# apple/ml-neuman

Hardware: AMD Instinct MI355X
Metric: rays_per_sec (800x800 frame, 128 samples/ray coarse + 128 importance, NeuMan background NeRF) (higher is better)
Workload: dtype coarse (sampling) pass: split-fp16 hi+lo MFMA x3, f32 accumulate; fine (shading) pass: per-row-scaled int16 as two int8 limbs on the i8 MFMA x3, exact int32 accumulate, encodings on split bf16

## Files before the change

ml-neuman_amd/csrc/mlp_device.h:

```cpp
#pragma once
#include "common.h"
#include "mlp_layout.h"
#include "mlp_launch.h"

namespace {

using nm::kTileM;

typedef __attribute__((ext_vector_type(8))) __bf16 bf16x8;
typedef __attribute__((ext_vector_type(2))) __bf16 bf16x2;
typedef __attribute__((ext_vector_type(8))) _Float16 f16x8;
typedef __attribute__((ext_vector_type(2))) _Float16 f16x2;

constexpr bool is_split(int prec) { return prec == NM_PREC_BF16X3 || prec == NM_PREC_FP16X3; }
constexpr float kF16ActScale = 32.f;
typedef __attribute__((ext_vector_type(2))) float f32x2;
typedef __attribute__((ext_vector_type(16))) float f32x16;

constexpr int kThreads = 512;
constexpr int kChunkU4 = 2 * kTileM;
constexpr int kLoU4 = kTileM;
constexpr int H_BASE = 0;
constexpr int P_BASE = nm::kHChunks * kChunkU4;
constexpr int LDS_U4 = P_BASE + nm::kPeChunks * kChunkU4;
// ... 17 lines not shown
    float* out;
    float* dbg;
    unsigned long long* prof;
    int64_t n;
    int S;
    int in_mode;
    const int* ray_idx;
    const int* n_rays_dev;
    int s0, S_total;
    int stop_stage;
    float sigma_scale;
    int sigma_only;
    PeSpec pos, dir;
    float* save_h;
    float* save_hv;
    unsigned* save_bits;
    uint4* save_h16;
    uint4* save_feat16;
    unsigned* save_hvbits;
    uint4* save_x0h;
    uint4* save_d0h;
};

__device__ __forceinline__ float pe_feature(int p, float x0, float x1, float x2, PeSpec spec, const float* __restrict__ tab) {
    const int m = p - 3;
    float a = 0.f;
    bool is_cos = false;
    if (p >= 3 && m < 6 * spec.nfreq) {
        if (spec.kind == NM_PE_POSENC) {
            const int b = m / 6, r = m - 6 * b;
            const int dim = r >= 3 ? r - 3 : r;
            const float xv = dim == 0 ? x0 : (dim == 1 ? x1 : x2);
            a = xv * tab[b];
            is_cos = r >= 3;
        } else {
            const int n3 = 3 * spec.nfreq;
            is_cos = m >= n3;
            const float* b = tab + 3 * (is_cos ? m - n3 : m);
            a = fmaf(x2, b[2], fmaf(x1, b[1], x0 * b[0]));
        }
    }
    float sv, cv;
    sincosf(a, &sv, &cv);
    if (p < 3) return p == 0 ? x0 : (p == 1 ? x1 : x2);
    if (m >= 6 * spec.nfreq) return 0.f;
    return is_cos ? cv : sv;
}

__device__ __forceinline__ int64_t sample_record(const MlpArgs& a, int64_t i) {
    if (a.in_mode >= 3) return a.ray_idx[i];
    if (a.in_mode != 2) return i;
    const int64_t j = i / a.S;
    return (int64_t)a.ray_idx[j] * a.S_total + a.s0 + (i - j * a.S);
}
__device__ __forceinline__ void sample_input(const MlpArgs& a, int64_t i, bool is_dir, float& x0, float& x1, float& x2) {
    if (a.in_mode == 0 || a.in_mode == 4) {
        if (a.in_mode == 4) i = a.ray_idx[i];
        const float* src = (is_dir ? a.dirs : a.pts) + i * 3;
        x0 = src[0]; x1 = src[1]; x2 = src[2];
        return;
    }
    int64_t r, zi;
    if (a.in_mode == 3) i = a.ray_idx[i];
    if (a.in_mode != 2) {
        r = i / a.S;
        zi = i;
    } else {
        const int64_t j = i / a.S;
        r = a.ray_idx[j];
        zi = r * a.S_total + a.s0 + (i - j * a.S);
    }
    const float* d = a.direction + r * 3;
    if (is_dir) {
        x0 = d[0]; x1 = d[1]; x2 = d[2];
    } else {
        const float zz = a.z[zi];
        const float* o = a.origin + r * 3;
        x0 = o[0] + d[0] * zz;
        x1 = o[1] + d[1] * zz;
        x2 = o[2] + d[2] * zz;
    }
}

template <bool RELU, bool F16 = false>
__device__ __forceinline__ void split8(const float* v, uint4& hi, uint4& lo, float scale = 1.f) {
    unsigned h[4], l[4];
#pragma unroll
    for (int p = 0; p < 4; ++p) {
        f32x2 a = {v[2 * p], v[2 * p + 1]};
        if (F16) {
            a.x = __builtin_amdgcn_fmed3f(a.x * scale, RELU ? 0.f : -65504.f, 65504.f);
            a.y = __builtin_amdgcn_fmed3f(a.y * scale, RELU ? 0.f : -65504.f, 65504.f);
            const f16x2 hb = __builtin_convertvector(a, f16x2);
            const f32x2 hf = __builtin_convertvector(hb, f32x2);
            const f32x2 r = {a.x - hf.x, a.y - hf.y};
            const f16x2 lb = __builtin_convertvector(r, f16x2);
            h[p] = __builtin_bit_cast(unsigned, hb);
            l[p] = __builtin_bit_cast(unsigned, lb);
            continue;
        }
        if (RELU) {
            a.x = fmaxf(a.x, 0.f);
            a.y = fmaxf(a.y, 0.f);
        }
        const bf16x2 hb = __builtin_convertvector(a, bf16x2);
        const f32x2 hf = __builtin_convertvector(hb, f32x2);
        const f32x2 r = {a.x - hf.x, a.y - hf.y};
        const bf16x2 lb = __builtin_convertvector(r, bf16x2);
        h[p] = __builtin_bit_cast(unsigned, hb);
        l[p] = __builtin_bit_cast(unsigned, lb);
    }
    hi = make_uint4(h[0], h[1], h[2], h[3]);
    lo = make_uint4(l[0], l[1], l[2], l[3]);
}

__device__ __forceinline__ bf16x8 as_bf16x8(uint4 v) { return __builtin_bit_cast(bf16x8, v); }

typedef __attribute__((vector_size(16))) unsigned int v4u;
__device__ __forceinline__ bf16x8 ld_w(__amdgpu_buffer_rsrc_t wsrc, int voff, int soff) {
    return __builtin_bit_cast(bf16x8, __builtin_amdgcn_raw_buffer_load_b128(wsrc, voff, soff, 0));
}

struct WPre {
    bf16x8 h[2], l[2];
};
template <int PREC>
__device__ __forceinline__ void w_prefetch(WPre& W, __amdgpu_buffer_rsrc_t wsrc, int voff, int soff) {
#pragma unroll
    for (int u = 0; u < 2; ++u) {
        W.h[u] = ld_w(wsrc, voff, soff + u * nm::kStepBytes);
        if (is_split(PREC)) W.l[u] = ld_w(wsrc, voff, soff + u * nm::kStepBytes + 1024);
    }
}

template <int MB, int PREC>
__device__ __forceinline__ void x_load(uint4 (&h)[MB], uint4 (&l)[MB], const uint4* ph) {
#pragma unroll
    for (int mb = 0; mb < MB; ++mb) {
        h[mb] = ph[mb * 32];
        if (is_split(PREC)) l[mb] = ph[kLoU4 + mb * 32];
    }
}
__device__ __forceinline__ f16x8 as_f16x8(uint4 v) { return __builtin_bit_cast(f16x8, v); }
template <int MB, int PREC>
__device__ __forceinline__ void mfma_step(f32x16 (&acc)[MB], bf16x8 wh, bf16x8 wl, const uint4 (&xh)[MB], const uint4 (&xl)[MB]) {
    if (PREC == NM_PREC_FP16X3) {
        const f16x8 fh = __builtin_bit_cast(f16x8, wh), fl = __builtin_bit_cast(f16x8, wl);
#pragma unroll
        for (int mb = 0; mb < MB; ++mb) acc[mb] = __builtin_amdgcn_mfma_f32_32x32x16_f16(fh, as_f16x8(xl[mb]), acc[mb], 0, 0, 0);
#pragma unroll
        for (int mb = 0; mb < MB; ++mb) acc[mb] = __builtin_amdgcn_mfma_f32_32x32x16_f16(fl, as_f16x8(xh[mb]), acc[mb], 0, 0, 0);
#pragma unroll
        for (int mb = 0; mb < MB; ++mb) acc[mb] = __builtin_amdgcn_mfma_f32_32x32x16_f16(fh, as_f16x8(xh[mb]), acc[mb], 0, 0, 0);
        return;
    }
    if (PREC == NM_PREC_BF16X3) {
#pragma unroll
        for (int mb = 0; mb < MB; ++mb) acc[mb] = __builtin_amdgcn_mfma_f32_32x32x16_bf16(wh, as_bf16x8(xl[mb]), acc[mb], 0, 0, 0);
#pragma unroll
        for (int mb = 0; mb < MB; ++mb) acc[mb] = __builtin_amdgcn_mfma_f32_32x32x16_bf16(wl, as_bf16x8(xh[mb]), acc[mb], 0, 0, 0);
    }
#pragma unroll
    for (int mb = 0; mb < MB; ++mb) acc[mb] = __builtin_amdgcn_mfma_f32_32x32x16_bf16(wh, as_bf16x8(xh[mb]), acc[mb], 0, 0, 0);
}
template <int MB, int PREC>
__device__ __forceinline__ void k_run(f32x16 (&acc)[MB], WPre& W, __amdgpu_buffer_rsrc_t wsrc, int voff, int soff, int next_soff,
// ... 211 lines not shown
```

ml-neuman_amd/csrc/mlp_f16t.hip:

```cpp
#include "mlp_i8as.h"
#include <stdio.h>
#include <stdlib.h>

namespace {

constexpr int kWavesF = 4;
constexpr int kTileF = kWavesF * kRows;
constexpr int kPosU4F = nm::kPeChunks * 2 * kRows;
constexpr int kPeF = kWavesF * kPosU4F;
constexpr int kStepU4F = nm::kStepBytes / 16;
constexpr int kSlotU4F = 16 * kStepU4F;
constexpr int kSlotsF = 3;
constexpr int kF16TabF = 2 * nm::kStages + 2;
constexpr int kTabU4F = (nm::kBiasFloats + kF16TabF + 3) / 4;
constexpr int kSigmaStepsF = 8 * 4 + 6 * 8 * 16 + 8 * 20 + 16;
static_assert((kPeF + kSlotsF * kSlotU4F + kTabU4F) * 16 <= 160 * 1024, "LDS plan exceeds the CU");

struct RingF {
    const char* src;
    const uint4* rd;
    unsigned lds0;
    int off;
    int slot;
};
__device__ __forceinline__ void ring_piece_f(const RingF& R, int off, int slot, int j) {
    glds16(R.src + off + j * (kWavesF * 1024), __builtin_amdgcn_readfirstlane(R.lds0 + slot * (kSlotU4F * 16) + j * (kWavesF * 1024)));
}

struct ArgsF {
    MlpArgs a;
    const uint4* stream;
    const float* bias16;
    unsigned* dbg;
    int dbg_stage;
    int64_t dbg_tile;
};

#ifdef NM_F16T_BODY
#include NM_F16T_BODY
#else
#include "mlp_f16t_body.h"
#endif

__global__ __launch_bounds__(kWavesF * 64) __attribute__((amdgpu_waves_per_eu(1, 1))) void nerf_sigma_f16t_kernel(const ArgsF A) {
    __shared__ uint4 lds[kPeF + kSlotsF * kSlotU4F + kTabU4F];
    const MlpArgs a = resolve_args(A.a);
    const int tid = threadIdx.x, lane = tid & 63;
    const int w = __builtin_amdgcn_readfirstlane(tid >> 6);
    const int g = lane >> 5, s = lane & 31;
    uint4* pw = lds + w * kPosU4F;
    RingF R;
    R.src = reinterpret_cast<const char*>(A.stream) + lane * 16 + w * 1024;
    R.rd = lds + kPeF + lane;
    R.lds0 = (unsigned)(uintptr_t)(lds + kPeF) + w * 1024;
    {
        float* lb = reinterpret_cast<float*>(lds + kPeF + kSlotsF * kSlotU4F);
        for (int i = tid; i < nm::kBiasFloats + kF16TabF; i += kWavesF * 64) lb[i] = A.bias16[i];
    }
    for (int i = lane; i < kPosU4F; i += 64) pw[i] = make_uint4(0, 0, 0, 0);
    __syncthreads();
    for (int j = 0; j < kF16tUnit0Pieces; ++j) ring_piece_f(R, 0, 0, j);
    for (int j = 0; j < kF16tUnit0Pieces; ++j) ring_piece_f(R, kF16tUnit0Pieces * 4096, 1, j);
    R.off = 2 * kF16tUnit0Pieces * 4096;
    if (kF16tUnit0Pieces == 4) asm volatile("s_waitcnt vmcnt(4)" ::: "memory");
    else if (kF16tUnit0Pieces == 3) asm volatile("s_waitcnt vmcnt(3)" ::: "memory");
    else asm volatile("s_waitcnt vmcnt(2)" ::: "memory");
    __syncthreads();
    R.slot = 1;
    const float os = A.bias16[nm::kBiasFloats + nm::kStages + 8];
    unsigned bias_lds = (unsigned)(uintptr_t)(lds + kPeF + kSlotsF * kSlotU4F) + 16 * g;
    asm volatile("" : "+v"(bias_lds));
    const unsigned tab_lds = (unsigned)(uintptr_t)(lds + kPeF + kSlotsF * kSlotU4F) + nm::kBiasFloats * 4;
    const int64_t ntiles = (a.n + kTileF - 1) / kTileF;
#pragma unroll 1
    for (int64_t tile = blockIdx.x; tile < ntiles; tile += gridDim.x) {
        const int64_t row0 = tile * kTileF + w * kRows;
        fill_pe_wave<true>(pw, false, a, row0, lane);
        sigma_stages_asm(A, a, R, pw, bias_lds, tab_lds, g, s, tid, tile, row0, os);
    }
    asm volatile("s_waitcnt vmcnt(0)" ::: "memory");
}

}

namespace nm {

int sigma_f16t_ndir() { return kF16tNdir; }

int launch_sigma_f16t(const MlpLaunch& L, const void* stream16t, int stream_ndir, const float* pts, const float* dirs, const float* origin, const float* direction,
                      const float* z, int64_t n, int S, int in_mode, float sigma_scale, float* out, hipStream_t stream, const MlpChunk* chunk,
                      float* dbg, int dbg_stage) {
    static_assert(kSigmaStepsF * kStepBytes == 976 * 2048, "stream length");
    NM_REQUIRE(stream_ndir == kF16tNdir, "nerf_sigma_f16t_kernel: the stream was cut for %d direct parts per k-step, the kernel is generated for %d", stream_ndir, kF16tNdir);
    ArgsF A;
    MlpArgs& a = A.a;
    a.ray_idx = chunk ? chunk->ray_idx : nullptr;
    a.n_rays_dev = chunk ? chunk->n_rays_dev : nullptr;
    a.s0 = chunk ? chunk->s0 : 0;
    a.S_total = chunk ? chunk->S_total : S;
    a.wpack = nullptr; a.bias = nullptr;
    a.petab = L.petab;
    a.pts = pts; a.dirs = dirs; a.origin = origin; a.direction = direction; a.z = z;
    a.out = out; a.dbg = nullptr; a.prof = nullptr; a.n = n; a.S = S; a.in_mode = in_mode; a.stop_stage = -2; a.sigma_scale = sigma_scale;
    a.sigma_only = 1;
    a.save_h = nullptr; a.save_hv = nullptr; a.save_bits = nullptr; a.save_h16 = nullptr; a.save_feat16 = nullptr; a.save_hvbits = nullptr; a.save_x0h = nullptr; a.save_d0h = nullptr;
    a.pos = PeSpec{L.pe_kind, L.pos_nfreq, L.pos_octaves};
    a.dir = PeSpec{L.pe_kind, L.dir_nfreq, L.dir_octaves};
    A.stream = reinterpret_cast<const uint4*>(stream16t);
    A.bias16 = L.bias16;
    A.dbg = reinterpret_cast<unsigned*>(dbg);
    A.dbg_stage = dbg ? dbg_stage % 100 : -1;
    A.dbg_tile = dbg ? (int64_t)(dbg_stage / 100) * 256 : -1;
    const int64_t ntiles = (n + kTileF - 1) / kTileF;
    int dev = 0, cus = 256;
    if (hipGetDevice(&dev) == hipSuccess) {
        int v = 0;
        if (hipDeviceGetAttribute(&v, hipDeviceAttributeMultiprocessorCount, dev) == hipSuccess && v > 0) cus = v;
    }
    const int grid = (int)(ntiles < cus ? ntiles : cus);
    hipLaunchKernelGGL(nerf_sigma_f16t_kernel, dim3(grid), dim3(kWavesF * 64), 0, stream, A);
    return check_launch("nerf_sigma_f16t_kernel");
}

}
```

ml-neuman_amd/csrc/mlp_i8as.h:

```cpp
#pragma once
#include "mlp_device.h"

namespace {

typedef __attribute__((ext_vector_type(4))) int i32x4;
typedef __attribute__((ext_vector_type(16))) int i32x16;
typedef __attribute__((ext_vector_type(2))) short i16x2;
typedef __attribute__((address_space(3))) const float lds_cfloat;
typedef __attribute__((ext_vector_type(4))) float vf4;
typedef __attribute__((address_space(3))) const vf4 lds_cvf4;

constexpr int kRows = 32;
struct Args8s {
    MlpArgs a;
    const float* consts8;
    const uint4* image8;
    nm::LiveList live;
};

__device__ __forceinline__ i32x4 as_i32x4(uint4 v) { return __builtin_bit_cast(i32x4, v); }

template <bool F16 = false>
__device__ __forceinline__ void fill_pe_wave(uint4* pw, bool is_dir, const MlpArgs& a, int64_t base_row, int lane) {
    const PeSpec spec = is_dir ? a.dir : a.pos;
    const float* tab = a.petab + (is_dir ? 96 : 0);
    unsigned short* hi = reinterpret_cast<unsigned short*>(pw);
    auto put = [&](int row, int p, float v, bool clamp = false) {
        const int off = ((p >> 3) * (2 * kRows) + row) * 8 + (p & 7);
        if (F16) {
            float sv = v * kF16ActScale;
            if (clamp) sv = __builtin_amdgcn_fmed3f(sv, -65504.f, 65504.f);
            const _Float16 hb = (_Float16)sv;
            const _Float16 lb = (_Float16)(sv - (float)hb);
            hi[off] = __builtin_bit_cast(unsigned short, hb);
            hi[off + kRows * 8] = __builtin_bit_cast(unsigned short, lb);
            return;
        }
        const bf16x2 hb = __builtin_convertvector((f32x2){v, 0.f}, bf16x2);
        const f32x2 hf = __builtin_convertvector(hb, f32x2);
        const bf16x2 lb = __builtin_convertvector((f32x2){v - hf.x, 0.f}, bf16x2);
        hi[off] = (unsigned short)(__builtin_bit_cast(unsigned, hb) & 0xffffu);
        hi[off + kRows * 8] = (unsigned short)(__builtin_bit_cast(unsigned, lb) & 0xffffu);
    };
    if (spec.octaves) {
#pragma unroll 1
        for (int round = 0; round < 2; ++round) {
            const int j = 2 * round + (lane >> 5), row = lane & 31;
            if (j > 2) break;
            int64_t i = base_row + row;
            if (i >= a.n) i = a.n - 1;
            float x0, x1, x2;
            sample_input(a, i, is_dir, x0, x1, x2);
            const float xj = j == 0 ? x0 : (j == 1 ? x1 : x2);
            const float a0 = spec.kind == NM_PE_POSENC ? xj * tab[0] : fmaf(x2, tab[3 * j + 2], fmaf(x1, tab[3 * j + 1], x0 * tab[3 * j]));
            put(row, j, xj);
            double sn, cs;
            sincos_f64((double)a0, sn, cs);
            const int n3 = 3 * spec.nfreq;
            for (int b = 0; b < spec.nfreq; ++b) {
                if (spec.kind == NM_PE_POSENC) { put(row, 3 + 6 * b + j, (float)sn); put(row, 3 + 6 * b + 3 + j, (float)cs); }
                else { put(row, 3 + 3 * b + j, (float)sn); put(row, 3 + n3 + 3 * b + j, (float)cs); }
                const double s2 = 2.0 * sn * cs, c2 = 1.0 - 2.0 * sn * sn;
                sn = s2; cs = c2;
            }
        }
    } else {
        const int nchunks = is_dir ? 4 : nm::kPeChunks;
        for (int item = lane; item < nchunks * kRows; item += 64) {
            const int c = item >> 5, row = item & 31;
            int64_t i = base_row + row;
            if (i >= a.n) i = a.n - 1;
            float x0, x1, x2;
            sample_input(a, i, is_dir, x0, x1, x2);
#pragma unroll
            for (int e = 0; e < 8; ++e) put(row, 8 * c + e, pe_feature(8 * c + e, x0, x1, x2, spec, tab), true);
        }
    }
}

struct X8 {
    uint4 h[8], l[8];
};

__device__ __forceinline__ void glds16(const void* gsrc, unsigned lds_dst) {
    unsigned keep;
    asm volatile("s_mov_b32 %0, m0\n\ts_mov_b32 m0, %2\n\ts_nop 0\n\tglobal_load_lds_dwordx4 %1, off\n\ts_mov_b32 m0, %0"
                 : "=&s"(keep) : "v"(gsrc), "s"(lds_dst) : "memory");
}
__device__ __forceinline__ void bias16(f32x16& f, lds_cfloat* bias_blk) {
#pragma unroll
    for (int q = 0; q < 4; ++q) {
        const vf4 bs = *(lds_cvf4*)(bias_blk + 8 * q);
        f[4 * q] = bs.x; f[4 * q + 1] = bs.y; f[4 * q + 2] = bs.z; f[4 * q + 3] = bs.w;
    }
}
__device__ __forceinline__ void dequant16(f32x16& f, const i32x16& t, float sx256, lds_cfloat* bias_blk) {
#pragma unroll
    for (int q = 0; q < 4; ++q) {
        const vf4 bs = *(lds_cvf4*)(bias_blk + 8 * q);
        const float bsv[4] = {bs.x, bs.y, bs.z, bs.w};
#pragma unroll
        for (int j = 0; j < 4; ++j) f[4 * q + j] = fmaf((float)t[4 * q + j], sx256, bsv[j]);
    }
}
template <bool RELU>
__device__ __forceinline__ float max16(float m, const f32x16& f) {
#pragma unroll
    for (int r = 0; r < 16; ++r) m = fmaxf(m, RELU ? f[r] : fabsf(f[r]));
    return m;
}
__device__ __forceinline__ float row_max(float m) {
    typedef __attribute__((ext_vector_type(2))) unsigned u32x2;
    const u32x2 sw = __builtin_amdgcn_permlane32_swap(__float_as_uint(m), __float_as_uint(m), false, false);
    return fmaxf(__uint_as_float(sw.x), __uint_as_float(sw.y));
}
template <bool RELU>
__device__ __forceinline__ void quant16(const f32x16& f, float inv, uint4& xh, uint4& xl) {
    i16x2 P[8], Y[8];
#pragma unroll
    for (int i = 0; i < 8; ++i) {
        float y0 = f[2 * i] * inv, y1 = f[2 * i + 1] * inv;
        if (RELU) {
            y0 = __builtin_amdgcn_fmed3f(y0, 0.f, 1.f);
            y1 = __builtin_amdgcn_fmed3f(y1, 0.f, 1.f);
        }
        const i16x2 p = __builtin_amdgcn_cvt_pknorm_i16(y0, y1);
        P[i] = p;
        Y[i] = p + (i16x2){128, 128};
    }
    unsigned lo[4], hi[4];
#pragma unroll
    for (int k = 0; k < 4; ++k) {
        lo[k] = __builtin_amdgcn_perm(__builtin_bit_cast(unsigned, P[2 * k + 1]), __builtin_bit_cast(unsigned, P[2 * k]), 0x06040200u);
        hi[k] = __builtin_amdgcn_perm(__builtin_bit_cast(unsigned, Y[2 * k + 1]), __builtin_bit_cast(unsigned, Y[2 * k]), 0x07050301u);
    }
    xh = make_uint4(hi[0], hi[1], hi[2], hi[3]);
    xl = make_uint4(lo[0], lo[1], lo[2], lo[3]);
}
__device__ __forceinline__ float inv_of(float M) { return M > 0.f ? ((float)nm::kFixedMax / 32767.f) * __builtin_amdgcn_rcpf(M) : 0.f; }
__device__ __forceinline__ float scale_of(float M) { return M > 0.f ? M * (1.f / (float)nm::kFixedMax) : 1.f; }

constexpr int kWaves = 8;
constexpr int kTile = kWaves * kRows;
constexpr int kPWaveU4 = nm::kPeChunks * 2 * kRows;
constexpr int kPeU4 = kWaves * kPWaveU4;
constexpr int kStepU4 = nm::kStepBytes / 16;
constexpr int kSlotU4 = 12 * kStepU4;
constexpr int kSlots = 3;
constexpr int kBiasU4 = (nm::kBiasFloats + 16 + 3) / 4;
__host__ __device__ constexpr int block_pieces(int nsteps) { return (2 * nsteps + kWaves - 1) / kWaves; }

template <class S>
struct RingT {
    const char* src;
    const uint4* rd;
    unsigned lds0;
    int off;
    int slot;
// ... 87 lines not shown
```

ml-neuman_amd/csrc/mlp_i8f.hip:

```cpp
#include "mlp_i8as.h"

namespace {

constexpr int kTrunkSteps = 8 * 4 + 7 * 8 * 8 + 8 * 4 + 8;
constexpr int kHeadSteps = 8 * 8 + 4 * 10 + 4;
struct TrunkStream {
    static __host__ __device__ constexpr int steps(int i) { return i < 8 ? 4 : 8; }
};
struct HeadStream {
    static __host__ __device__ constexpr int steps(int i) {
        i = i >= 13 ? i - 13 : i;
        return i < 8 ? 8 : i < 12 ? 10 : 4;
    }
};

struct ArgsF {
    MlpArgs a;
    const float* consts8;
    const char* image;
    int head_off;
    char* list;
    int* tiles;
};

struct RingF {
    const char* src;
    const uint4* rd;
    unsigned lds0;
    int off, slot;
    int refill, np, nsteps2;
    int edge, next;
};
__device__ __forceinline__ void ring_piece(const RingF& R, int off, int slot, int j) {
    glds16(R.src + off + j * (kWaves * 1024), __builtin_amdgcn_readfirstlane(R.lds0 + slot * (kSlotU4 * 16) + j * (kWaves * 1024)));
}
template <class S>
__device__ __forceinline__ const uint4* ring_enter_f(RingF& R, int i) {
    const int np1 = block_pieces(S::steps(i + 1));
    if (np1 == 1) asm volatile("s_waitcnt vmcnt(1)" ::: "memory");
    else if (np1 == 2) asm volatile("s_waitcnt vmcnt(2)" ::: "memory");
    else asm volatile("s_waitcnt vmcnt(3)" ::: "memory");
    __builtin_amdgcn_s_barrier();
    const uint4* cur = R.rd + R.slot * kSlotU4;
    R.refill = R.slot == 0 ? kSlots - 1 : R.slot - 1;
    R.slot = R.slot == kSlots - 1 ? 0 : R.slot + 1;
    R.np = block_pieces(S::steps(i + 2));
    R.nsteps2 = S::steps(i + 2);
    return cur;
}
__device__ __forceinline__ void ring_copy(RingF& R, int j) {
    if (j < R.np) ring_piece(R, R.off, R.refill, j);
    if (j == R.np - 1) {
        R.off += R.nsteps2 * nm::kStepBytes;
        if (R.off == R.edge) R.off = R.next;
    }
}

__global__ __launch_bounds__(kWaves * 64, 2) void nerf_mlp_i8s_fused_kernel(const ArgsF A) {
    __shared__ uint4 lds[kPeU4 + kSlots * kSlotU4 + kBiasU4];
    __shared__ float units[4];
    __shared__ unsigned appended;
    const MlpArgs a = A.a;
    const int tid = threadIdx.x, lane = tid & 63;
    const int w = __builtin_amdgcn_readfirstlane(tid >> 6);
    const int g = lane >> 5, s = lane & 31;
    uint4* pw = lds + w * kPWaveU4;
    RingF R;
    R.src = A.image + lane * 16 + w * 1024;
    R.rd = lds + kPeU4 + lane;
    R.lds0 = (unsigned)(uintptr_t)(lds + kPeU4) + w * 1024;
    R.slot = 0;
    {
        float* lb = reinterpret_cast<float*>(lds + kPeU4 + kSlots * kSlotU4);
        for (int i = tid; i < nm::kBiasFloats + 16; i += kWaves * 64) lb[i] = A.consts8[nm::kBiasFloats + i];
    }
    if (tid == 0) appended = 0;
    if (tid < 4) units[tid] = A.consts8[tid == 0 ? nm::stage_b_off(8) + 256 : nm::stage_b_off(10) + tid - 1];
    __syncthreads();
    ring_piece(R, 0, 0, 0);
    ring_piece(R, 4 * nm::kStepBytes, 1, 0);
    const float* kappa = reinterpret_cast<const float*>(lds + kPeU4 + kSlots * kSlotU4) + nm::kBiasFloats;
    unsigned bias_lds = (unsigned)(uintptr_t)(lds + kPeU4 + kSlots * kSlotU4) + 16 * g;
    asm volatile("" : "+v"(bias_lds));
    lds_cfloat* bias = (lds_cfloat*)(uintptr_t)bias_lds;
    const int64_t ntiles = (a.n + kTile - 1) / kTile;
    for (int i = lane; i < kPWaveU4; i += 64) pw[i] = make_uint4(0, 0, 0, 0);
    char* const mine = A.list + (int64_t)blockIdx.x * nm::kFusedListBytes;
    uint4* const lx = reinterpret_cast<uint4*>(mine);
    float* const lsx = reinterpret_cast<float*>(mine + nm::kFusedEntries * 512);
    int* const lidx = reinterpret_cast<int*>(mine + nm::kFusedEntries * 516);

    int64_t tile = blockIdx.x;
    unsigned consumed = 0;
    int head = 0, ntrunk = 0, nhead = 0;
#pragma unroll 1
    for (;;) {
        __builtin_amdgcn_fence(__ATOMIC_RELEASE, "workgroup");
        __builtin_amdgcn_s_barrier();
        __builtin_amdgcn_fence(__ATOMIC_ACQUIRE, "workgroup");
        const unsigned pending = (unsigned)__builtin_amdgcn_readfirstlane(__hip_atomic_load(&appended, __ATOMIC_RELAXED, __HIP_MEMORY_SCOPE_WORKGROUP)) - consumed;
        if (head && pending == 0) break;
        const unsigned ntake = head ? (pending < (unsigned)kTile ? pending : (unsigned)kTile) : 0u;
        const bool more = (head ? tile : tile + gridDim.x) < ntiles;
        const int next_head = pending - ntake >= (unsigned)kTile || !more;
        R.off = head ? A.head_off + 16 * nm::kStepBytes : 8 * nm::kStepBytes;
        R.edge = head ? A.head_off + kHeadSteps * nm::kStepBytes : kTrunkSteps * nm::kStepBytes;
        R.next = next_head ? A.head_off : kTrunkSteps * nm::kStepBytes;
        asm volatile("" : "+s"(R.off), "+s"(R.edge), "+s"(R.next));
        if (!head) {
            const int64_t row0 = tile * kTile + w * kRows;
            fill_pe_wave(pw, false, a, row0, lane);
            X8 X;
            float sx;
            {
                f32x16 f[8];
                float m = 0.f;
#pragma unroll
                for (int b = 0; b < 8; ++b) {
                    const uint4* ws = ring_enter_f<TrunkStream>(R, b);
                    bias16(f[b], bias + nm::stage_b_off(0) + 32 * b);
                    k_bf<4, true>(f[b], pw, g, s, ws, &R);
                    m = max16<true>(m, f[b]);
                }
                const float M = row_max(m), inv = inv_of(M);
#pragma unroll
                for (int b = 0; b < 8; ++b) quant16<true>(f[b], inv, X.h[b], X.l[b]);
                sx = scale_of(M);
            }
#pragma unroll 1
            for (int st = 1; st <= 7; ++st) {
                const float sxin = sx * (256.f * kappa[st]);
                const int i0 = 8 * st + (st > 5 ? 4 : 0);
                f32x16 f[8];
                float m = 0.f;
                i32x16 tp;
#pragma unroll
                for (int b = 0; b < 8; ++b) {
                    const uint4* ws = ring_enter_f<TrunkStream>(R, i0 + b);
                    if (b == 0) {
                        k_i8<8>(tp, X, ws, R);
                    } else {
                        i32x16 t;
                        k_i8_impl<8, true>(t, X, ws, R, f[b - 1], tp, bias + 256 * st + 32 * (b - 1), sxin, m);
                        tp = t;
                    }
                }
                dequant16(f[7], tp, sxin, bias + 256 * st + 32 * 7);
                if (st == 5) {
#pragma unroll
                    for (int u = 0; u < 4; ++u) {
                        const uint4* ws = ring_enter_f<TrunkStream>(R, 48 + u);
                        k_bf<4, true>(f[2 * u], pw, g, s, ws, &R, 0);
                        k_bf<4, true>(f[2 * u + 1], pw, g, s, ws + 4 * kStepU4, &R, 2);
                    }
                    m = 0.f;
#pragma unroll
                    for (int b = 0; b < 7; ++b) m = max16<true>(m, f[b]);
                }
                m = max16<true>(m, f[7]);
                const float M = row_max(m), inv = inv_of(M);
#pragma unroll
                for (int b = 0; b < 8; ++b) quant16<true>(f[b], inv, X.h[b], X.l[b]);
                sx = scale_of(M);
            }
            {
                i32x16 t;
                f32x16 fa;
                k_i8<8>(t, X, ring_enter_f<TrunkStream>(R, 68), R);
                dequant16(fa, t, sx * (256.f * kappa[8]), bias + nm::stage_b_off(8) + 256);
                const float sigma = fa[0] * units[0];
                const float v = sigma * a.sigma_scale;
                int sb = s, gb = g;
                asm volatile("" : "+v"(sb), "+v"(gb));
                const int64_t i = row0 + s;
                if (g == 0 && i < a.n) reinterpret_cast<float4*>(a.out)[i] = make_float4(0.f, 0.f, 0.f, v);
                const unsigned live = (unsigned)__builtin_amdgcn_ballot_w64(g == 0 && i < a.n && !(v <= 0.f));
                if (live) {
                    unsigned base = 0;
                    if (lane == 0) base = __hip_atomic_fetch_add(&appended, (unsigned)__builtin_popcount(live), __ATOMIC_RELAXED, __HIP_MEMORY_SCOPE_WORKGROUP);
                    base = (unsigned)__builtin_amdgcn_readfirstlane(base);
                    if ((live >> sb) & 1) {
                        const unsigned e = (base + __builtin_popcount(live & ((1u << sb) - 1u))) % (unsigned)nm::kFusedEntries;
                        uint4* dst = lx + gb * nm::kFusedEntries + e;
#pragma unroll
                        for (int k = 0; k < 8; ++k) {
                            dst[(4 * k) * nm::kFusedEntries] = X.h[k];
                            dst[(4 * k + 2) * nm::kFusedEntries] = X.l[k];
                        }
                        if (g == 0) { lsx[e] = sx; lidx[e] = (int)i; }
                    }
                }
            }
            tile += gridDim.x;
            ++ntrunk;
        } else {
            const unsigned e0 = consumed % (unsigned)nm::kFusedEntries;
            MlpArgs ah = a;
            ah.in_mode = 3;
            ah.ray_idx = lidx + e0;
            ah.n = ntake;
            ah.s0 = 0;
            ah.S_total = a.S;
            const int64_t row0 = w * kRows;
            int e = w * kRows + s;
            const bool listed = e < (int)ntake;
            if (!listed) e = (int)ntake - 1;
            X8 X;
            {
                const uint4* src = lx + g * nm::kFusedEntries + e0 + e;
#pragma unroll
                for (int k = 0; k < 8; ++k) {
                    X.h[k] = src[(4 * k) * nm::kFusedEntries];
                    X.l[k] = src[(4 * k + 2) * nm::kFusedEntries];
                }
            }
            float sx = lsx[e0 + e];
            int rec = lidx[e0 + e];
            fill_pe_wave(pw, true, ah, row0, lane);
            asm volatile("" : "+v"(rec));
            {
                const float sxin = sx * (256.f * kappa[8]);
                f32x16 f[8];
                float m = 0.f;
#pragma unroll
                for (int b = 0; b < 8; ++b) {
                    i32x16 t;
                    k_i8<8>(t, X, ring_enter_f<HeadStream>(R, b), R);
                    dequant16(f[b], t, sxin, bias + nm::stage_b_off(8) + 32 * b);
                    m = max16<false>(m, f[b]);
                }
                const float M = row_max(m), inv = inv_of(M);
#pragma unroll
                for (int b = 0; b < 8; ++b) quant16<false>(f[b], inv, X.h[b], X.l[b]);
                sx = scale_of(M);
            }
            {
                const float sxin = sx * (256.f * kappa[9]);
                f32x16 f[4];
                float m = 0.f;
#pragma unroll
                for (int b = 0; b < 4; ++b) {
                    i32x16 t;
                    const uint4* ws = ring_enter_f<HeadStream>(R, 8 + b);
                    k_i8<8>(t, X, ws, R);
                    dequant16(f[b], t, sxin, bias + nm::stage_b_off(9) + 32 * b);
                    k_bf<2>(f[b], pw, g, s, ws + 8 * kStepU4);
                    m = max16<true>(m, f[b]);
                }
                const float M = row_max(m), inv = inv_of(M);
#pragma unroll
                for (int b = 0; b < 4; ++b) quant16<true>(f[b], inv, X.h[b], X.l[b]);
                sx = scale_of(M);
            }
            {
                i32x16 t;
                f32x16 fr;
                k_i8<4>(t, X, ring_enter_f<HeadStream>(R, 12), R);
                dequant16(fr, t, sx * (256.f * kappa[10]), bias + nm::stage_b_off(10));
                if (g == 0 && listed) {
                    float* o = a.out + (int64_t)rec * 4;
                    o[0] = fr[0] * units[1]; o[1] = fr[1] * units[2]; o[2] = fr[2] * units[3];
                }
            }
            consumed += ntake;
            ++nhead;
        }
        head = next_head;
    }
    if (tid == 0) { A.tiles[2 * blockIdx.x] = ntrunk; A.tiles[2 * blockIdx.x + 1] = nhead; }
    asm volatile("s_waitcnt vmcnt(0)" ::: "memory");
}

}

namespace nm {

int launch_mlp_i8f(const MlpLaunch& L, const void* trunk8, int head_off, const float* origin, const float* direction, const float* z, int64_t n, int S,
                   float sigma_scale, float* out, void* workspace, hipStream_t stream) {
    ArgsF A;
    MlpArgs& a = A.a;
    a.ray_idx = nullptr; a.n_rays_dev = nullptr; a.s0 = 0; a.S_total = S;
    a.wpack = nullptr; a.bias = nullptr;
    a.petab = L.petab;
    a.pts = nullptr; a.dirs = nullptr; a.origin = origin; a.direction = direction; a.z = z;
    a.out = out; a.dbg = nullptr; a.prof = nullptr; a.n = n; a.S = S; a.in_mode = 1; a.stop_stage = -2; a.sigma_scale = sigma_scale;
    a.sigma_only = 0;
    a.save_h = nullptr; a.save_hv = nullptr; a.save_bits = nullptr; a.save_h16 = nullptr; a.save_feat16 = nullptr; a.save_hvbits = nullptr; a.save_x0h = nullptr; a.save_d0h = nullptr;
    a.pos = PeSpec{L.pe_kind, L.pos_nfreq, L.pos_octaves};
    a.dir = PeSpec{L.pe_kind, L.dir_nfreq, L.dir_octaves};
    A.consts8 = L.consts8;
    A.image = static_cast<const char*>(trunk8);
    A.head_off = head_off;
    const int64_t groups = fused_groups(n);
    A.list = static_cast<char*>(workspace);
    A.tiles = reinterpret_cast<int*>(A.list + groups * kFusedListBytes);
    int dev = 0, cus = kFusedMaxGroups;
    if (hipGetDevice(&dev) == hipSuccess) {
        int v = 0;
        if (hipDeviceGetAttribute(&v, hipDeviceAttributeMultiprocessorCount, dev) == hipSuccess && v > 0) cus = v;
    }
    const int grid = (int)(groups < cus ? groups : cus);
// ... 6 lines not shown
```

ml-neuman_amd/csrc/mlp_i8h.hip:

```cpp
#include "mlp_i8as.h"

namespace {

constexpr int kHeadBlocks = 13;
constexpr int kHeadSteps = 8 * 8 + 4 * 10 + 4;
struct HeadStream {
    static __host__ __device__ constexpr int steps(int i) {
        i = i >= kHeadBlocks ? i - kHeadBlocks : i;
        return i < 8 ? 8 : i < 12 ? 10 : 4;
    }
    static constexpr int kBytes = kHeadSteps * nm::kStepBytes;
};
typedef RingT<HeadStream> Ring;

__global__ __launch_bounds__(kWaves * 64, 2) void nerf_head_i8s_kernel(const Args8s A) {
    __shared__ uint4 lds[kPeU4 + kSlots * kSlotU4 + kBiasU4];
    const MlpArgs a = resolve_args(A.a);
    const int tid = threadIdx.x, lane = tid & 63;
    const int w = __builtin_amdgcn_readfirstlane(tid >> 6);
    const int g = lane >> 5, s = lane & 31;
    uint4* pw = lds + w * kPWaveU4;
    Ring R;
    R.src = reinterpret_cast<const char*>(A.image8) + lane * 16 + w * 1024;
    R.rd = lds + kPeU4 + lane;
    R.lds0 = (unsigned)(uintptr_t)(lds + kPeU4) + w * 1024;
    R.off = 0;
    R.slot = 0;
    {
        float* lb = reinterpret_cast<float*>(lds + kPeU4 + kSlots * kSlotU4);
        for (int i = tid; i < nm::kBiasFloats + 16; i += kWaves * 64) lb[i] = A.consts8[nm::kBiasFloats + i];
    }
    __syncthreads();
    ring_piece(R, 0, 0, 0);
    ring_piece(R, 0, 0, 1);
    ring_piece(R, HeadStream::steps(0) * nm::kStepBytes, 1, 0);
    ring_piece(R, HeadStream::steps(0) * nm::kStepBytes, 1, 1);
    R.off = (HeadStream::steps(0) + HeadStream::steps(1)) * nm::kStepBytes;
    const float u_r = A.consts8[nm::stage_b_off(10)], u_g = A.consts8[nm::stage_b_off(10) + 1], u_b = A.consts8[nm::stage_b_off(10) + 2];
    const float* kappa = reinterpret_cast<const float*>(lds + kPeU4 + kSlots * kSlotU4) + nm::kBiasFloats;
    unsigned bias_lds = (unsigned)(uintptr_t)(lds + kPeU4 + kSlots * kSlotU4) + 16 * g;
    asm volatile("" : "+v"(bias_lds));
    lds_cfloat* bias = (lds_cfloat*)(uintptr_t)bias_lds;
    const int64_t ntiles = (a.n + kTile - 1) / kTile;
    for (int i = lane; i < kPWaveU4; i += 64) pw[i] = make_uint4(0, 0, 0, 0);

#pragma unroll 1
    for (int64_t tile = blockIdx.x; tile < ntiles; tile += gridDim.x) {
        const int64_t row0 = tile * kTile + w * kRows;
        asm volatile("" : "+s"(R.off));
        int64_t e = row0 + s;
        const bool mine = e < a.n;
        if (!mine) e = a.n - 1;
        X8 X;
        {
            const uint4* src = A.live.x + g * A.live.cap + e;
#pragma unroll
            for (int k = 0; k < 8; ++k) {
                X.h[k] = src[(4 * k) * A.live.cap];
                X.l[k] = src[(4 * k + 2) * A.live.cap];
            }
        }
        float sx = A.live.sx[e];
        const int rec = A.live.idx[e];
        fill_pe_wave(pw, true, a, row0, lane);
        {
            const float sxin = sx * (256.f * kappa[8]);
            f32x16 f[8];
            float m = 0.f;
#pragma unroll
            for (int b = 0; b < 8; ++b) {
                i32x16 t;
                k_i8<8>(t, X, ring_enter(R, b), R);
                dequant16(f[b], t, sxin, bias + nm::stage_b_off(8) + 32 * b);
                m = max16<false>(m, f[b]);
            }
            const float M = row_max(m), inv = inv_of(M);
#pragma unroll
            for (int b = 0; b < 8; ++b) quant16<false>(f[b], inv, X.h[b], X.l[b]);
            sx = scale_of(M);
        }
        {
            const float sxin = sx * (256.f * kappa[9]);
            f32x16 f[4];
            float m = 0.f;
#pragma unroll
            for (int b = 0; b < 4; ++b) {
                i32x16 t;
                const uint4* ws = ring_enter(R, 8 + b);
                k_i8<8>(t, X, ws, R);
                dequant16(f[b], t, sxin, bias + nm::stage_b_off(9) + 32 * b);
                k_bf<2>(f[b], pw, g, s, ws + 8 * kStepU4);
                m = max16<true>(m, f[b]);
            }
            const float M = row_max(m), inv = inv_of(M);
#pragma unroll
            for (int b = 0; b < 4; ++b) quant16<true>(f[b], inv, X.h[b], X.l[b]);
            sx = scale_of(M);
        }
        {
            i32x16 t;
            f32x16 fr;
            k_i8<4>(t, X, ring_enter(R, 12), R);
            dequant16(fr, t, sx * (256.f * kappa[10]), bias + nm::stage_b_off(10));
            if (g == 0 && mine) {
                float* o = a.out + (int64_t)rec * 4;
                o[0] = fr[0] * u_r; o[1] = fr[1] * u_g; o[2] = fr[2] * u_b;
            }
        }
    }
    asm volatile("s_waitcnt vmcnt(0)" ::: "memory");
}

}

namespace nm {

int launch_mlp_i8h(const MlpLaunch& L, const void* head8, int in_mode, const float* dirs, const float* direction, int S_total, const LiveList& live,
                   int64_t max_entries, float* out, hipStream_t stream) {
    Args8s A;
    MlpArgs& a = A.a;
    a.ray_idx = live.idx;
    a.n_rays_dev = live.count;
    a.s0 = 0;
    a.S_total = S_total;
    a.wpack = nullptr; a.bias = nullptr;
    a.petab = L.petab;
    a.pts = nullptr; a.dirs = dirs; a.origin = nullptr; a.direction = direction; a.z = nullptr;
    a.out = out; a.dbg = nullptr; a.prof = nullptr; a.n = max_entries; a.S = S_total; a.in_mode = in_mode; a.stop_stage = -2; a.sigma_scale = 1.f;
    a.sigma_only = 0;
    a.save_h = nullptr; a.save_hv = nullptr; a.save_bits = nullptr; a.save_h16 = nullptr; a.save_feat16 = nullptr; a.save_hvbits = nullptr; a.save_x0h = nullptr; a.save_d0h = nullptr;
    a.pos = PeSpec{L.pe_kind, L.pos_nfreq, L.pos_octaves};
    a.dir = PeSpec{L.pe_kind, L.dir_nfreq, L.dir_octaves};
    A.consts8 = L.consts8;
    A.image8 = reinterpret_cast<const uint4*>(head8);
    A.live = live;
    const int64_t ntiles = (max_entries + kTile - 1) / kTile;
    int dev = 0, cus = 256;
    if (hipGetDevice(&dev) == hipSuccess) {
        int v = 0;
        if (hipDeviceGetAttribute(&v, hipDeviceAttributeMultiprocessorCount, dev) == hipSuccess && v > 0) cus = v;
    }
    const int grid = (int)(ntiles < cus ? ntiles : cus);
    hipLaunchKernelGGL(nerf_head_i8s_kernel, dim3(grid), dim3(kWaves * 64), 0, stream, A);
    return check_launch("nerf_head_i8s_kernel");
}

}
// ... 1 lines not shown
```

ml-neuman_amd/csrc/mlp_i8s.hip:

```cpp
#include "mlp_i8as.h"

namespace {

constexpr int kTileBlocks = 82;
__host__ __device__ constexpr int block_steps(int i) {
    i = i >= kTileBlocks ? i - kTileBlocks : i;
    return i < 8 ? 4 : i < 77 ? 8 : i < 81 ? 10 : 4;
}
struct TileStream {
    static __host__ __device__ constexpr int steps(int i) { return block_steps(i); }
    static constexpr int kBytes = (int)nm::kWeightBytes8;
};
typedef RingT<TileStream> Ring;

enum { WHOLE = 0, PLAIN = 1, TRUNK = 2 };
template <int MODE>
__global__ __launch_bounds__(kWaves * 64, 2) void nerf_mlp_i8s_kernel(const Args8s A) {
    __shared__ uint4 lds[kPeU4 + kSlots * kSlotU4 + kBiasU4];
    const MlpArgs a = resolve_args(A.a);
    const int tid = threadIdx.x, lane = tid & 63;
    const int w = __builtin_amdgcn_readfirstlane(tid >> 6);
    const int g = lane >> 5, s = lane & 31;
    uint4* pw = lds + w * kPWaveU4;
    Ring R;
    R.src = reinterpret_cast<const char*>(A.image8) + lane * 16 + w * 1024;
    R.rd = lds + kPeU4 + lane;
    R.lds0 = (unsigned)(uintptr_t)(lds + kPeU4) + w * 1024;
    R.off = 0;
    R.slot = 0;
    {
        float* lb = reinterpret_cast<float*>(lds + kPeU4 + kSlots * kSlotU4);
        for (int i = tid; i < nm::kBiasFloats + 16; i += kWaves * 64) lb[i] = A.consts8[nm::kBiasFloats + i];
    }
    __syncthreads();
    ring_piece(R, 0, 0, 0);
    ring_piece(R, block_steps(0) * nm::kStepBytes, 1, 0);
    R.off = (block_steps(0) + block_steps(1)) * nm::kStepBytes;
    const float u_sigma = A.consts8[nm::stage_b_off(8) + 256];
    const float u_r = A.consts8[nm::stage_b_off(10)], u_g = A.consts8[nm::stage_b_off(10) + 1], u_b = A.consts8[nm::stage_b_off(10) + 2];
    const float* kappa = reinterpret_cast<const float*>(lds + kPeU4 + kSlots * kSlotU4) + nm::kBiasFloats;
    unsigned bias_lds = (unsigned)(uintptr_t)(lds + kPeU4 + kSlots * kSlotU4) + 16 * g;
    asm volatile("" : "+v"(bias_lds));
    lds_cfloat* bias = (lds_cfloat*)(uintptr_t)bias_lds;
    const int64_t ntiles = (a.n + kTile - 1) / kTile;
    for (int i = lane; i < kPWaveU4; i += 64) pw[i] = make_uint4(0, 0, 0, 0);

#pragma unroll 1
    for (int64_t tile = blockIdx.x; tile < ntiles; tile += gridDim.x) {
        const int64_t row0 = tile * kTile + w * kRows;
        fill_pe_wave(pw, false, a, row0, lane);
        X8 X;
        float sx;
        {
            f32x16 f[8];
            float m = 0.f;
#pragma unroll
            for (int b = 0; b < 8; ++b) {
                const uint4* ws = ring_enter(R, b);
                bias16(f[b], bias + nm::stage_b_off(0) + 32 * b);
                k_bf<4, true>(f[b], pw, g, s, ws, &R);
                m = max16<true>(m, f[b]);
            }
            const float M = row_max(m), inv = inv_of(M);
#pragma unroll
            for (int b = 0; b < 8; ++b) quant16<true>(f[b], inv, X.h[b], X.l[b]);
            sx = scale_of(M);
        }
#pragma unroll 1
        for (int st = 1; st <= 7; ++st) {
            const float sxin = sx * (256.f * kappa[st]);
            const int i0 = 8 * st + (st > 5 ? 4 : 0);
            f32x16 f[8];
            float m = 0.f;
            i32x16 tp;
#pragma unroll
            for (int b = 0; b < 8; ++b) {
                const uint4* ws = ring_enter(R, i0 + b);
                if (b == 0) {
                    k_i8<8>(tp, X, ws, R);
                } else {
                    i32x16 t;
                    k_i8_impl<8, true>(t, X, ws, R, f[b - 1], tp, bias + 256 * st + 32 * (b - 1), sxin, m);
                    tp = t;
                }
            }
            dequant16(f[7], tp, sxin, bias + 256 * st + 32 * 7);
            if (st == 5) {
#pragma unroll
                for (int u = 0; u < 4; ++u) {
                    const uint4* ws = ring_enter(R, 48 + u);
                    k_bf<4, true>(f[2 * u], pw, g, s, ws, &R, 0);
                    k_bf<4, true>(f[2 * u + 1], pw, g, s, ws + 4 * kStepU4, &R, 2);
                }
                m = 0.f;
#pragma unroll
                for (int b = 0; b < 7; ++b) m = max16<true>(m, f[b]);
            }
            m = max16<true>(m, f[7]);
            const float M = row_max(m), inv = inv_of(M);
#pragma unroll
            for (int b = 0; b < 8; ++b) quant16<true>(f[b], inv, X.h[b], X.l[b]);
            sx = scale_of(M);
            if (st == 5 && !(MODE != WHOLE && a.sigma_only == MODE + 1)) {
                fill_pe_wave(pw, true, a, row0, lane);
            }
        }
        if (MODE == PLAIN && a.sigma_only == 2) {
            i32x16 t;
            f32x16 fo;
            k_i8<8>(t, X, ring_enter(R, 68), R);
            dequant16(fo, t, sx * (256.f * kappa[8]), bias + nm::stage_b_off(8) + 256);
            const float* up = A.consts8 + nm::stage_b_off(8) + 256;
            const int64_t i = row0 + s;
            if (g == 0 && i < a.n)
                reinterpret_cast<float4*>(a.out)[sample_record(a, i)] = make_float4(fo[0] * up[0], fo[1] * up[1], fo[2] * up[2], fo[3] * up[3] * a.sigma_scale);
            R.off = (block_steps(0) + block_steps(1)) * nm::kStepBytes;
            continue;
        }
        if (MODE == TRUNK && a.sigma_only == 3) {
            i32x16 t;
            f32x16 fa;
            k_i8<8>(t, X, ring_enter(R, 68), R);
            dequant16(fa, t, sx * (256.f * kappa[8]), bias + nm::stage_b_off(8) + 256);
            const float sigma = fa[0] * u_sigma;
            const float v = sigma * a.sigma_scale;
            const int64_t i = row0 + s;
            const int64_t rec = g == 0 && i < a.n ? sample_record(a, i) : 0;
            if (g == 0 && i < a.n) reinterpret_cast<float4*>(a.out)[rec] = make_float4(0.f, 0.f, 0.f, v);
            const unsigned live = (unsigned)__builtin_amdgcn_ballot_w64(g == 0 && i < a.n && !(v <= 0.f));
            if (live) {
                int base = 0;
                if (lane == 0) base = atomicAdd(A.live.count, __builtin_popcount(live));
                base = __builtin_amdgcn_readfirstlane(base);
                if ((live >> s) & 1) {
                    const int64_t e = base + __builtin_popcount(live & ((1u << s) - 1u));
                    uint4* dst = A.live.x + g * A.live.cap + e;
#pragma unroll
                    for (int k = 0; k < 8; ++k) {
                        dst[(4 * k) * A.live.cap] = X.h[k];
                        dst[(4 * k + 2) * A.live.cap] = X.l[k];
                    }
                    if (g == 0) { A.live.sx[e] = sx; A.live.idx[e] = (int)rec; }
                }
            }
            R.off = (block_steps(0) + block_steps(1)) * nm::kStepBytes;
            continue;
        }
        float sigma;
        {
            const float sxin = sx * (256.f * kappa[8]);
            {
                i32x16 t;
                f32x16 fa;
                k_i8<8>(t, X, ring_enter(R, 68), R);
                dequant16(fa, t, sxin, bias + nm::stage_b_off(8) + 256);
                sigma = fa[0] * u_sigma;
            }
            f32x16 f[8];
            float m = 0.f;
#pragma unroll
            for (int b = 0; b < 8; ++b) {
                i32x16 t;
                k_i8<8>(t, X, ring_enter(R, 69 + b), R);
                dequant16(f[b], t, sxin, bias + nm::stage_b_off(8) + 32 * b);
                m = max16<false>(m, f[b]);
            }
            const float M = row_max(m), inv = inv_of(M);
#pragma unroll
            for (int b = 0; b < 8; ++b) quant16<false>(f[b], inv, X.h[b], X.l[b]);
            sx = scale_of(M);
        }
        {
            const float sxin = sx * (256.f * kappa[9]);
            f32x16 f[4];
            float m = 0.f;
#pragma unroll
            for (int b = 0; b < 4; ++b) {
                i32x16 t;
                const uint4* ws = ring_enter(R, 77 + b);
                k_i8<8>(t, X, ws, R);
                dequant16(f[b], t, sxin, bias + nm::stage_b_off(9) + 32 * b);
                k_bf<2>(f[b], pw, g, s, ws + 8 * kStepU4);
                m = max16<true>(m, f[b]);
            }
            const float M = row_max(m), inv = inv_of(M);
#pragma unroll
            for (int b = 0; b < 4; ++b) quant16<true>(f[b], inv, X.h[b], X.l[b]);
// ... 55 lines not shown
```

Baseline: 1.524 million.

## Rebalance positional-encoding fill across wave halves and stage PE tables in LDS

The per-wave positional-encoding fill now computes each row's sample input once per lane, using 32-bit division for the ray/sample split instead of repeated int64 divides. The third axis's octave chain is split across both wave halves: the second half jumps ahead by repeated angle doubling, so neither half sits idle in the second round. The PE frequency tables are copied into a small LDS array at kernel start in every MLP kernel, and the store offset is computed with a cheaper multiply. The cost is extra LDS, redundant doubling steps in the second half, and more index logic in a path that is small next to the MFMA stages.

```diff
diff --git a/ml-neuman_amd/csrc/mlp_device.h b/ml-neuman_amd/csrc/mlp_device.h
--- a/ml-neuman_amd/csrc/mlp_device.h
+++ b/ml-neuman_amd/csrc/mlp_device.h
@@ -123,6 +123,38 @@
     }
 }
 
+__device__ __forceinline__ void sample_input_rows(const MlpArgs& a, int64_t base_row, int row, bool is_dir, float& x0, float& x1, float& x2) {
+    if (a.in_mode != 1 && a.in_mode != 2) {
+        int64_t i = base_row + row;
+        if (i >= a.n) i = a.n - 1;
+        sample_input(a, i, is_dir, x0, x1, x2);
+        return;
+    }
+    const int64_t last = a.n - 1;
+    const int64_t b = base_row < last ? base_row : last;
+    const int64_t q0 = b / a.S;
+    const unsigned rem0 = (unsigned)(b - q0 * a.S);
+    const int64_t room = last - b;
+    const unsigned rowc = room < (int64_t)row ? (unsigned)room : (unsigned)row;
+    const unsigned t = rem0 + rowc;
+    const unsigned dq = t / (unsigned)a.S, s = t - dq * (unsigned)a.S;
+    int64_t r = q0 + dq, zi = b + rowc;
+    if (a.in_mode == 2) {
+        r = a.ray_idx[q0 + dq];
+        zi = r * a.S_total + a.s0 + s;
+    }
+    const float* d = a.direction + r * 3;
+    if (is_dir) {
+        x0 = d[0]; x1 = d[1]; x2 = d[2];
+    } else {
+        const float zz = a.z[zi];
+        const float* o = a.origin + r * 3;
+        x0 = o[0] + d[0] * zz;
+        x1 = o[1] + d[1] * zz;
+        x2 = o[2] + d[2] * zz;
+    }
+}
+
 template <bool RELU, bool F16 = false>
 __device__ __forceinline__ void split8(const float* v, uint4& hi, uint4& lo, float scale = 1.f) {
     unsigned h[4], l[4];
diff --git a/ml-neuman_amd/csrc/mlp_f16t.hip b/ml-neuman_amd/csrc/mlp_f16t.hip
--- a/ml-neuman_amd/csrc/mlp_f16t.hip
+++ b/ml-neuman_amd/csrc/mlp_f16t.hip
@@ -14,7 +14,7 @@
 constexpr int kF16TabF = 2 * nm::kStages + 2;
 constexpr int kTabU4F = (nm::kBiasFloats + kF16TabF + 3) / 4;
 constexpr int kSigmaStepsF = 8 * 4 + 6 * 8 * 16 + 8 * 20 + 16;
-static_assert((kPeF + kSlotsF * kSlotU4F + kTabU4F) * 16 <= 160 * 1024, "LDS plan exceeds the CU");
+static_assert((kPeF + kSlotsF * kSlotU4F + kTabU4F) * 16 + kPeTabFloats * 4 <= 160 * 1024, "LDS plan exceeds the CU");
 
 struct RingF {
     const char* src;
@@ -44,6 +44,7 @@
 
 __global__ __launch_bounds__(kWavesF * 64) __attribute__((amdgpu_waves_per_eu(1, 1))) void nerf_sigma_f16t_kernel(const ArgsF A) {
     __shared__ uint4 lds[kPeF + kSlotsF * kSlotU4F + kTabU4F];
+    __shared__ float petab_l[kPeTabFloats];
     const MlpArgs a = resolve_args(A.a);
     const int tid = threadIdx.x, lane = tid & 63;
     const int w = __builtin_amdgcn_readfirstlane(tid >> 6);
@@ -57,6 +58,7 @@
         float* lb = reinterpret_cast<float*>(lds + kPeF + kSlotsF * kSlotU4F);
         for (int i = tid; i < nm::kBiasFloats + kF16TabF; i += kWavesF * 64) lb[i] = A.bias16[i];
     }
+    pe_tables_to_lds(petab_l, a, tid, kWavesF * 64);
     for (int i = lane; i < kPosU4F; i += 64) pw[i] = make_uint4(0, 0, 0, 0);
     __syncthreads();
     for (int j = 0; j < kF16tUnit0Pieces; ++j) ring_piece_f(R, 0, 0, j);
@@ -75,7 +77,7 @@
 #pragma unroll 1
     for (int64_t tile = blockIdx.x; tile < ntiles; tile += gridDim.x) {
         const int64_t row0 = tile * kTileF + w * kRows;
-        fill_pe_wave<true>(pw, false, a, row0, lane);
+        fill_pe_wave<true>(pw, false, a, row0, lane, petab_l);
         sigma_stages_asm(A, a, R, pw, bias_lds, tab_lds, g, s, tid, tile, row0, os);
     }
     asm volatile("s_waitcnt vmcnt(0)" ::: "memory");
diff --git a/ml-neuman_amd/csrc/mlp_i8as.h b/ml-neuman_amd/csrc/mlp_i8as.h
--- a/ml-neuman_amd/csrc/mlp_i8as.h
+++ b/ml-neuman_amd/csrc/mlp_i8as.h
@@ -20,13 +20,19 @@
 
 __device__ __forceinline__ i32x4 as_i32x4(uint4 v) { return __builtin_bit_cast(i32x4, v); }
 
+constexpr int kPeTabFloats = 192;
+__device__ __forceinline__ void pe_tables_to_lds(float* tabs, const MlpArgs& a, int tid, int nthreads) {
+    for (int i = tid; i < kPeTabFloats; i += nthreads) tabs[i] = a.petab[i];
+}
 template <bool F16 = false>
-__device__ __forceinline__ void fill_pe_wave(uint4* pw, bool is_dir, const MlpArgs& a, int64_t base_row, int lane) {
+__device__ __forceinline__ void fill_pe_wave(uint4* pw, bool is_dir, const MlpArgs& a, int64_t base_row, int lane, const float* tabs) {
     const PeSpec spec = is_dir ? a.dir : a.pos;
-    const float* tab = a.petab + (is_dir ? 96 : 0);
+    const float* tab = tabs + (is_dir ? 96 : 0);
     unsigned short* hi = reinterpret_cast<unsigned short*>(pw);
-    auto put = [&](int row, int p, float v, bool clamp = false) {
-        const int off = ((p >> 3) * (2 * kRows) + row) * 8 + (p & 7);
+    const int row = lane & 31, half = lane >> 5;
+    const int rb = row * 8;
+    auto put = [&](int p, float v, bool clamp = false) {
+        const int off = rb + p + (int)__umul24((unsigned)p >> 3, 2 * kRows * 8 - 8);
         if (F16) {
             float sv = v * kF16ActScale;
             if (clamp) sv = __builtin_amdgcn_fmed3f(sv, -65504.f, 65504.f);
@@ -42,38 +48,41 @@
         hi[off] = (unsigned short)(__builtin_bit_cast(unsigned, hb) & 0xffffu);
         hi[off + kRows * 8] = (unsigned short)(__builtin_bit_cast(unsigned, lb) & 0xffffu);
     };
+    float x0, x1, x2;
+    sample_input_rows(a, base_row, row, is_dir, x0, x1, x2);
     if (spec.octaves) {
+        const int nf = spec.nfreq, h = (nf + 1) >> 1, n3 = 3 * nf;
 #pragma unroll 1
         for (int round = 0; round < 2; ++round) {
-            const int j = 2 * round + (lane >> 5), row = lane & 31;
-            if (j > 2) break;
-            int64_t i = base_row + row;
-            if (i >= a.n) i = a.n - 1;
-            float x0, x1, x2;
-            sample_input(a, i, is_dir, x0, x1, x2);
+            const int j = round ? 2 : half;
+            const int nst = round ? h : nf;
+            const int b0 = round && half ? nf - h : 0;
             const float xj = j == 0 ? x0 : (j == 1 ? x1 : x2);
             const float a0 = spec.kind == NM_PE_POSENC ? xj * tab[0] : fmaf(x2, tab[3 * j + 2], fmaf(x1, tab[3 * j + 1], x0 * tab[3 * j]));
-            put(row, j, xj);
+            if (b0 == 0) put(j, xj);
             double sn, cs;
             sincos_f64((double)a0, sn, cs);
-            const int n3 = 3 * spec.nfreq;
-            for (int b = 0; b < spec.nfreq; ++b) {
-                if (spec.kind == NM_PE_POSENC) { put(row, 3 + 6 * b + j, (float)sn); put(row, 3 + 6 * b + 3 + j, (float)cs); }
-                else { put(row, 3 + 3 * b + j, (float)sn); put(row, 3 + n3 + 3 * b + j, (float)cs); }
+            if (round) {
+                for (int b = 0; b < nf - h; ++b) {
+                    const double s2 = 2.0 * sn * cs, c2 = 1.0 - 2.0 * sn * sn;
+                    if (half) { sn = s2; cs = c2; }
+                }
+            }
+            int ps = spec.kind == NM_PE_POSENC ? 3 + 6 * b0 + j : 3 + 3 * b0 + j;
+            const int dp = spec.kind == NM_PE_POSENC ? 6 : 3, pc = spec.kind == NM_PE_POSENC ? 3 : n3;
+            for (int b = 0; b < nst; ++b, ps += dp) {
+                put(ps, (float)sn);
+                put(ps + pc, (float)cs);
                 const double s2 = 2.0 * sn * cs, c2 = 1.0 - 2.0 * sn * sn;
                 sn = s2; cs = c2;
             }
         }
     } else {
+        const float* gtab = a.petab + (is_dir ? 96 : 0);
         const int nchunks = is_dir ? 4 : nm::kPeChunks;
-        for (int item = lane; item < nchunks * kRows; item += 64) {
-            const int c = item >> 5, row = item & 31;
-            int64_t i = base_row + row;
-            if (i >= a.n) i = a.n - 1;
-            float x0, x1, x2;
-            sample_input(a, i, is_dir, x0, x1, x2);
-#pragma unroll
-            for (int e = 0; e < 8; ++e) put(row, 8 * c + e, pe_feature(8 * c + e, x0, x1, x2, spec, tab), true);
+        for (int c = half; c < nchunks; c += 2) {
+#pragma unroll
+            for (int e = 0; e < 8; ++e) put(8 * c + e, pe_feature(8 * c + e, x0, x1, x2, spec, gtab), true);
         }
     }
 }
diff --git a/ml-neuman_amd/csrc/mlp_i8f.hip b/ml-neuman_amd/csrc/mlp_i8f.hip
--- a/ml-neuman_amd/csrc/mlp_i8f.hip
+++ b/ml-neuman_amd/csrc/mlp_i8f.hip
@@ -58,6 +58,7 @@
 
 __global__ __launch_bounds__(kWaves * 64, 2) void nerf_mlp_i8s_fused_kernel(const ArgsF A) {
     __shared__ uint4 lds[kPeU4 + kSlots * kSlotU4 + kBiasU4];
+    __shared__ float petab_l[kPeTabFloats];
     __shared__ float units[4];
     __shared__ unsigned appended;
     const MlpArgs a = A.a;
@@ -74,6 +75,7 @@
         float* lb = reinterpret_cast<float*>(lds + kPeU4 + kSlots * kSlotU4);
         for (int i = tid; i < nm::kBiasFloats + 16; i += kWaves * 64) lb[i] = A.consts8[nm::kBiasFloats + i];
     }
+    pe_tables_to_lds(petab_l, a, tid, kWaves * 64);
     if (tid == 0) appended = 0;
     if (tid < 4) units[tid] = A.consts8[tid == 0 ? nm::stage_b_off(8) + 256 : nm::stage_b_off(10) + tid - 1];
     __syncthreads();
@@ -109,7 +111,7 @@
         asm volatile("" : "+s"(R.off), "+s"(R.edge), "+s"(R.next));
         if (!head) {
             const int64_t row0 = tile * kTile + w * kRows;
-            fill_pe_wave(pw, false, a, row0, lane);
+            fill_pe_wave(pw, false, a, row0, lane, petab_l);
             X8 X;
             float sx;
             {
@@ -216,7 +218,7 @@
             }
             float sx = lsx[e0 + e];
             int rec = lidx[e0 + e];
-            fill_pe_wave(pw, true, ah, row0, lane);
+            fill_pe_wave(pw, true, ah, row0, lane, petab_l);
             asm volatile("" : "+v"(rec));
             {
                 const float sxin = sx * (256.f * kappa[8]);
diff --git a/ml-neuman_amd/csrc/mlp_i8h.hip b/ml-neuman_amd/csrc/mlp_i8h.hip
--- a/ml-neuman_amd/csrc/mlp_i8h.hip
+++ b/ml-neuman_amd/csrc/mlp_i8h.hip
@@ -15,6 +15,7 @@
 
 __global__ __launch_bounds__(kWaves * 64, 2) void nerf_head_i8s_kernel(const Args8s A) {
     __shared__ uint4 lds[kPeU4 + kSlots * kSlotU4 + kBiasU4];
+    __shared__ float petab_l[kPeTabFloats];
     const MlpArgs a = resolve_args(A.a);
     const int tid = threadIdx.x, lane = tid & 63;
     const int w = __builtin_amdgcn_readfirstlane(tid >> 6);
@@ -30,6 +31,7 @@
         float* lb = reinterpret_cast<float*>(lds + kPeU4 + kSlots * kSlotU4);
         for (int i = tid; i < nm::kBiasFloats + 16; i += kWaves * 64) lb[i] = A.consts8[nm::kBiasFloats + i];
     }
+    pe_tables_to_lds(petab_l, a, tid, kWaves * 64);
     __syncthreads();
     ring_piece(R, 0, 0, 0);
     ring_piece(R, 0, 0, 1);
@@ -62,7 +64,7 @@
         }
         float sx = A.live.sx[e];
         const int rec = A.live.idx[e];
-        fill_pe_wave(pw, true, a, row0, lane);
+        fill_pe_wave(pw, true, a, row0, lane, petab_l);
         {
             const float sxin = sx * (256.f * kappa[8]);
             f32x16 f[8];
diff --git a/ml-neuman_amd/csrc/mlp_i8s.hip b/ml-neuman_amd/csrc/mlp_i8s.hip
--- a/ml-neuman_amd/csrc/mlp_i8s.hip
+++ b/ml-neuman_amd/csrc/mlp_i8s.hip
@@ -17,6 +17,7 @@
 template <int MODE>
 __global__ __launch_bounds__(kWaves * 64, 2) void nerf_mlp_i8s_kernel(const Args8s A) {
     __shared__ uint4 lds[kPeU4 + kSlots * kSlotU4 + kBiasU4];
+    __shared__ float petab_l[kPeTabFloats];
     const MlpArgs a = resolve_args(A.a);
     const int tid = threadIdx.x, lane = tid & 63;
     const int w = __builtin_amdgcn_readfirstlane(tid >> 6);
@@ -32,6 +33,7 @@
         float* lb = reinterpret_cast<float*>(lds + kPeU4 + kSlots * kSlotU4);
         for (int i = tid; i < nm::kBiasFloats + 16; i += kWaves * 64) lb[i] = A.consts8[nm::kBiasFloats + i];
     }
+    pe_tables_to_lds(petab_l, a, tid, kWaves * 64);
     __syncthreads();
     ring_piece(R, 0, 0, 0);
     ring_piece(R, block_steps(0) * nm::kStepBytes, 1, 0);
@@ -48,7 +50,7 @@
 #pragma unroll 1
     for (int64_t tile = blockIdx.x; tile < ntiles; tile += gridDim.x) {
         const int64_t row0 = tile * kTile + w * kRows;
-        fill_pe_wave(pw, false, a, row0, lane);
+        fill_pe_wave(pw, false, a, row0, lane, petab_l);
         X8 X;
         float sx;
         {
@@ -102,7 +104,7 @@
             for (int b = 0; b < 8; ++b) quant16<true>(f[b], inv, X.h[b], X.l[b]);
             sx = scale_of(M);
             if (st == 5 && !(MODE != WHOLE && a.sigma_only == MODE + 1)) {
-                fill_pe_wave(pw, true, a, row0, lane);
+                fill_pe_wave(pw, true, a, row0, lane, petab_l);
             }
         }
         if (MODE == PLAIN && a.sigma_only == 2) {
```

After: 1.530 million, median of 6. Within noise of the previous version (+0.4%).
